# samholt/ODE-Discovery-for-Longitudinal-Heterogeneous-Treatment-Effects-Inference

Measured on AMD Instinct MI355X. Metric: patient-trajectories/sec (N×T RK4 steps) at 1/2/4/8 GPUs; RMSE vs CPU ref, higher is better.
Workload: dtype f64; 1 GPU; C2: PK/PD 100k patients/GPU x 200 steps fp64 - discovery (savgol+FD4+poly2 library+Gram, STLSQ) + RK4 counterfactual rollout; mode=deferred

## Files before the change

ode-discovery-for-longitudinal-heterogeneous-treatment-effects-inference_amd/csrc/insite_common.h:

```cpp
#pragma once
#include <hip/hip_runtime.h>

#include <cstdint>

#include "insite_hip.h"

namespace {

constexpr int kWave = 64;
constexpr int kWavesPerBlock = 4;
constexpr int kBlock = kWave * kWavesPerBlock;

#define SGC(a, b, c, d, e, den) a / den, b / den, c / den, d / den, e / den
__device__ __forceinline__ double dot5(double w0, double w1, double w2, double w3, double w4,
                                       double a, double b, double c, double d, double e) {
  return w0 * a + w1 * b + w2 * c + w3 * d + w4 * e;
}

__device__ __forceinline__ double sg_interior(double a, double b, double c, double d, double e) {
  return dot5(SGC(-3.0, 12.0, 17.0, 12.0, -3.0, 35.0), a, b, c, d, e);
}
__device__ __forceinline__ double sg_pos0(double a, double b, double c, double d, double e) {
  return dot5(SGC(69.0, 4.0, -6.0, 4.0, -1.0, 70.0), a, b, c, d, e);
}
__device__ __forceinline__ double sg_pos1(double a, double b, double c, double d, double e) {
  return dot5(SGC(2.0, 27.0, 12.0, -8.0, 2.0, 35.0), a, b, c, d, e);
}
__device__ __forceinline__ double sg_pos3(double a, double b, double c, double d, double e) {
  return dot5(SGC(2.0, -8.0, 12.0, 27.0, 2.0, 35.0), a, b, c, d, e);
}
__device__ __forceinline__ double sg_pos4(double a, double b, double c, double d, double e) {
  return dot5(SGC(-1.0, 4.0, -6.0, 4.0, 69.0, 70.0), a, b, c, d, e);
}
__device__ __forceinline__ double fd_interior(double a, double b, double , double d, double e) {
  return (1.0 / 12.0) * a + (-2.0 / 3.0) * b + (2.0 / 3.0) * d + (-1.0 / 12.0) * e;
}
__device__ __forceinline__ double fd_pos0(double a, double b, double c, double d, double e) {
  return dot5(-25.0 / 12.0, 4.0, -3.0, 4.0 / 3.0, -0.25, a, b, c, d, e);
}
__device__ __forceinline__ double fd_pos1(double a, double b, double c, double d, double e) {
  return dot5(-0.25, -5.0 / 6.0, 1.5, -0.5, 1.0 / 12.0, a, b, c, d, e);
}
__device__ __forceinline__ double fd_pos3(double a, double b, double c, double d, double e) {
  return dot5(-1.0 / 12.0, 0.5, -1.5, 5.0 / 6.0, 0.25, a, b, c, d, e);
}
__device__ __forceinline__ double fd_pos4(double a, double b, double c, double d, double e) {
  return dot5(0.25, -4.0 / 3.0, 3.0, -4.0, 25.0 / 12.0, a, b, c, d, e);
}

__device__ __forceinline__ void wave_lds_sync() {
  __builtin_amdgcn_fence(__ATOMIC_SEQ_CST, "wavefront");
  __builtin_amdgcn_wave_barrier();
  __builtin_amdgcn_fence(__ATOMIC_SEQ_CST, "wavefront");
}

__device__ __forceinline__ int wave_min_i(int v) {
#pragma unroll
  for (int off = 32; off > 0; off >>= 1) v = min(v, __shfl_xor(v, off, kWave));
  return __builtin_amdgcn_readfirstlane(v);
}
__device__ __forceinline__ int wave_max_i(int v) {
#pragma unroll
  for (int off = 32; off > 0; off >>= 1) v = max(v, __shfl_xor(v, off, kWave));
  return __builtin_amdgcn_readfirstlane(v);
}

__device__ __forceinline__ unsigned bit_transpose32(unsigned x, int lane) {
  const unsigned m[5] = {0x0000FFFFu, 0x00FF00FFu, 0x0F0F0F0Fu, 0x33333333u, 0x55555555u};
#pragma unroll
  for (int k = 0; k < 5; ++k) {
    const int sh = 16 >> k;
    const unsigned y = (unsigned)__shfl_xor((int)x, sh, kWave);
    x = (lane & sh) ? ((x & ~m[k]) | ((y >> sh) & m[k])) : ((x & m[k]) | ((y << sh) & ~m[k]));
  }
  return x;
}

struct GramW {
  double sg0, sg1, sg2;
  double fd1, fd2;
  double inv_dt;
};

__device__ __forceinline__ double sg_int(const GramW& w, double a, double b, double c, double d, double e) {
  return w.sg0 * c + w.sg1 * (b + d) + w.sg2 * (a + e);
}
__device__ __forceinline__ double fd_int(const GramW& w, double a, double b, double d, double e) {
  return w.fd1 * (d - b) + w.fd2 * (e - a);
}

typedef double dbl4 __attribute__((ext_vector_type(4)));
constexpr unsigned kOOB = 0x80000000u;

typedef unsigned int u32x4 __attribute__((ext_vector_type(4)));
typedef unsigned int u32x2 __attribute__((ext_vector_type(2)));

struct StlsqParams {
  double thr, alpha;
  int32_t max_iter, unbias, enabled;
};


#ifndef INSITE_STORE_AUX
#define INSITE_STORE_AUX 2
#endif
constexpr int kStoreAux = INSITE_STORE_AUX;

inline int32_t launch_status() { return hipGetLastError() == hipSuccess ? INSITE_OK : INSITE_E_HIP; }

}
```

ode-discovery-for-longitudinal-heterogeneous-treatment-effects-inference_amd/csrc/insite_hip.hip:

```cpp
#include <hip/hip_runtime.h>
#include <type_traits>

#include <cmath>
#include <cstdint>
#include <atomic>
#include <cstring>

#include "insite_hip.h"
#include "insite_irregular.h"
#include "insite_affine.h"

namespace {

constexpr int kGramMaxBlocks = 1024;
constexpr int kPsStride = 17;

#ifdef INSITE_TIMING
constexpr int kTsWaves = 1 << 16, kTsSlots = 10;
__device__ unsigned long long g_tstamp[kTsWaves * kTsSlots];
#define INSITE_TSTAMP(wave, slot)                                                                   \
  do {                                                                                              \
    const unsigned long long t_ = __builtin_amdgcn_s_memtime();                                     \
    if ((threadIdx.x & 63) == 0 && (wave) < kTsWaves) g_tstamp[(int64_t)(wave) * kTsSlots + (slot)] = t_; \
  } while (0)
// ... 28 lines not shown
  int8_t ex[INSITE_MAX_TERMS];
  int8_t eu[INSITE_MAX_TERMS][INSITE_MAX_STATICS];
  int8_t ei[kMaxEntries];
  int8_t ek[kMaxEntries];
  int32_t mfma;
  int32_t nq;
  int32_t n_atoms;
  int8_t atom_exp[16][INSITE_MAX_STATICS];
  int8_t col_atom[INSITE_MAX_TERMS];
  int8_t qatom[16];
  int8_t qmom[16];
  int8_t qcol[kMaxEntries];
  int32_t ucode[INSITE_MAX_TERMS];
  int32_t acode[16];
};

__device__ __forceinline__ double monomial(const LibDesc& lib, int j, const double* u) {
  return monomial_code(lib.ucode[j] & 0xffffff, u);
}
__device__ __forceinline__ int col_ex(const LibDesc& lib, int j) { return (lib.ucode[j] >> 24) & 0xff; }

#ifndef INSITE_GT
#define INSITE_GT 16
#endif
#ifndef INSITE_PF
#define INSITE_PF 1
#endif
constexpr int kGT = INSITE_GT;
constexpr int kGStride = kGT + 1;
constexpr int kGSlot = kGStride > 17 ? kGStride : 17;
constexpr int kGPF = INSITE_PF;
#ifndef INSITE_GRAM_SCPF
#define INSITE_GRAM_SCPF 1
#endif
#ifndef INSITE_TM_DEPTH
#define INSITE_TM_DEPTH 2
#endif
constexpr int kTmDepth = INSITE_TM_DEPTH;

__device__ __forceinline__ void add_row(double xk, double dk, double& Sx, double& Sxx, double& Sd, double& Sdx) {
  Sx += xk;
  Sxx = fma(xk, xk, Sxx);
  Sd += dk;
  Sdx = fma(dk, xk, Sdx);
}

template <int LL>
__device__ void small_trajectory(const double* __restrict__ xrow, int64_t step, const GramW& w, double& Sx,
                                 double& Sxx, double& Sd, double& Sdx) {
  double xv[LL], xs[LL];
#pragma unroll
  for (int j = 0; j < LL; ++j) xv[j] = xrow[j * step];
#pragma unroll
  for (int k = 0; k < LL; ++k) {
    if (k == 0) xs[k] = sg_pos0(xv[0], xv[1], xv[2], xv[3], xv[4]);
    else if (k == 1) xs[k] = sg_pos1(xv[0], xv[1], xv[2], xv[3], xv[4]);
    else if (k == LL - 2) xs[k] = sg_pos3(xv[LL - 5], xv[LL - 4], xv[LL - 3], xv[LL - 2], xv[LL - 1]);
    else if (k == LL - 1) xs[k] = sg_pos4(xv[LL - 5], xv[LL - 4], xv[LL - 3], xv[LL - 2], xv[LL - 1]);
    else xs[k] = sg_int(w, xv[k - 2], xv[k - 1], xv[k], xv[k + 1], xv[k + 2]);
  }
#pragma unroll
  for (int k = 0; k < LL; ++k) {
    double d;
    if (k == 0) d = fd_pos0(xs[0], xs[1], xs[2], xs[3], xs[4]) * w.inv_dt;
    else if (k == 1) d = fd_pos1(xs[0], xs[1], xs[2], xs[3], xs[4]) * w.inv_dt;
    else if (k == LL - 2) d = fd_pos3(xs[LL - 5], xs[LL - 4], xs[LL - 3], xs[LL - 2], xs[LL - 1]) * w.inv_dt;
    else if (k == LL - 1) d = fd_pos4(xs[LL - 5], xs[LL - 4], xs[LL - 3], xs[LL - 2], xs[LL - 1]) * w.inv_dt;
    else d = fd_int(w, xs[k - 2], xs[k - 1], xs[k + 1], xs[k + 2]);
    add_row(xv[k], d, Sx, Sxx, Sd, Sdx);
  }
}


__device__ __forceinline__ void tele_hi(const GramW& w, double vm1, double v0, double v1, double v2, double& sd,
                                        double& sdx) {
  sd = w.fd1 * (v1 + v0) + w.fd2 * ((v2 + v1) + (v0 + vm1));
  sdx = w.fd1 * (v0 * v1) + w.fd2 * (vm1 * v1 + v0 * v2);
}
__device__ __forceinline__ void tele_lo(const GramW& w, double vm2, double vm1, double v0, double v1, double& sd,
                                        double& sdx) {
  sd = w.fd1 * (v0 + vm1) + w.fd2 * ((v1 + v0) + (vm1 + vm2));
  sdx = w.fd1 * (vm1 * v0) + w.fd2 * (vm2 * v0 + vm1 * v1);
}

#ifndef INSITE_TAIL_RELEASE_FENCE
#define INSITE_TAIL_RELEASE_FENCE 0
#endif
constexpr int kTailGroup = 16;
constexpr int kTailMaxGroups = 64;
constexpr int kTailMaxEnt = INSITE_MAX_ARMS * (INSITE_MAX_TERMS * (INSITE_MAX_TERMS + 1) / 2 + INSITE_MAX_TERMS);
struct GramOut {
  double* G;
  double* b;
  int n_arms;
  double* coef;
  int8_t* mask;
  int32_t* iters;
  StlsqParams sp;
  double* mom;
};

template <int F>
__device__ int stlsq_solve(const double (&g)[F][F], const double (&rhs)[F], double thr, double alpha,
                           int max_iter, int unbias, double (&c)[F], unsigned& sup,
                           unsigned init = (1u << F) - 1u);

__device__ __forceinline__ void tail_store(double* p, double v) {
  __hip_atomic_store(reinterpret_cast<unsigned long long*>(p), __double_as_longlong(v), __ATOMIC_RELAXED,
                     __HIP_MEMORY_SCOPE_AGENT);
}

template <int STF>
__device__ __forceinline__ void tail_finish(double* red, int n_ent, const LibDesc& lib, const GramOut& o) {
  const int64_t F = lib.F;
  double* dense = red + kTailMaxEnt + 8;
  constexpr int kDense = STF * STF + STF;
  for (int idx = threadIdx.x; idx < n_ent; idx += kBlock) {
    const int a = idx / lib.nE, e = idx - a * lib.nE;
    const int i = lib.ei[e], k = lib.ek[e];
    const double v = red[idx];
    if (k >= 0) {
      o.G[(a * F + i) * F + k] = v;
      o.G[(a * F + k) * F + i] = v;
      if constexpr (STF > 0) {
        dense[a * kDense + i * STF + k] = v;
        dense[a * kDense + k * STF + i] = v;
      }
    } else {
      o.b[a * F + i] = v;
      if constexpr (STF > 0) dense[a * kDense + STF * STF + i] = v;
    }
  }
  if constexpr (STF > 0) {
    __syncthreads();
    const int a = (int)threadIdx.x;
    if (a < o.n_arms) {
      const double* d = dense + a * kDense;
      double g[STF][STF], rhs[STF], c[STF];
#pragma unroll
      for (int i = 0; i < STF; ++i) {
        rhs[i] = d[STF * STF + i];
#pragma unroll
        for (int j = 0; j <= i; ++j) g[i][j] = d[i * STF + j];
      }
      unsigned sup = 0u;
      const int it = stlsq_solve<STF>(g, rhs, o.sp.thr, o.sp.alpha, o.sp.max_iter, o.sp.unbias, c, sup);
#pragma unroll
      for (int i = 0; i < STF; ++i) {
        o.coef[a * STF + i] = c[i];
        if (o.mask) o.mask[a * STF + i] = (int8_t)((sup >> i) & 1u);
      }
      if (o.iters) o.iters[a] = it;
    }
  }
}

template <int STF>
__device__ __forceinline__ void gram_tail(const int vblk, const int nblk, double* __restrict__ part, int n_ent,
                                          unsigned* __restrict__ cnt, const LibDesc& lib, const GramOut& o,
                                          double* red) {
  int* flag = reinterpret_cast<int*>(red + kTailMaxEnt);
  const int tg = nblk <= kTailGroup * kTailMaxGroups
                     ? kTailGroup
                     : ((nblk + kTailMaxGroups - 1) / kTailMaxGroups + kTailGroup - 1) / kTailGroup * kTailGroup;
  const int ng = (nblk + tg - 1) / tg;
  const int g = vblk / tg;
// ... 139 lines not shown
          const double2 v = *reinterpret_cast<const double2*>(q);
          vx[j] = v.x;
          vy[j] = v.y;
        } else {
          vx[j] = q[0];
          vy[j] = odd_last ? 0.0 : q[1];
        }
      }
#pragma unroll
      for (int j = 0; j < kDynUnroll; ++j) {
        ax += r + j < r1 ? vx[j] : 0.0;
        ay += r + j < r1 ? vy[j] : 0.0;
      }
    }
    gsum[gq * 2 * npair + 2 * pp] = ax;
    gsum[gq * 2 * npair + 2 * pp + 1] = ay;
  }
  __syncthreads();
  for (int q = t; q < n_ent; q += kBlock) {
    double acc = 0.0;
    for (int g = 0; g < ngr; ++g) acc += gsum[g * 2 * npair + q];
    red[q] = acc;
  }
  __syncthreads();
  tail_finish<STF>(red, n_ent, lib, o);
}
static_assert(kTailMaxEnt + 8 + INSITE_MAX_ARMS * (INSITE_MAX_TERMS * INSITE_MAX_TERMS + INSITE_MAX_TERMS) +
                      2 * kBlock + 64 <= kWavesPerBlock * kWave * kGSlot,
              "dyn_finalize's group sums fit the gram kernel's LDS array");
static_assert(kTailMaxEnt + 8 + INSITE_MAX_ARMS * (INSITE_MAX_TERMS * INSITE_MAX_TERMS + INSITE_MAX_TERMS) <=
                  kWavesPerBlock * kWave * kGSlot,
              "tail scratch fits the gram kernel's LDS array");

constexpr int kGramSmem = kWavesPerBlock * kWave * kGSlot;
#ifndef INSITE_GRAM_ORDER
#define INSITE_GRAM_ORDER 0
#endif
#ifndef INSITE_GRAM_LOAD_AUX
#define INSITE_GRAM_LOAD_AUX 0
#endif
__device__ __forceinline__ int64_t gram_item_tile(int64_t item, int n_seg, int64_t n_tiles) {
  return INSITE_GRAM_ORDER ? item % n_tiles : item / n_seg;
}
__device__ __forceinline__ int gram_item_seg(int64_t item, int n_seg, int64_t n_tiles) {
  return INSITE_GRAM_ORDER ? (int)(item / n_tiles) : (int)(item - (item / n_seg) * n_seg);
}
template <bool MFMA, int NARM>
__device__ __forceinline__ void gram_block_partial(const int vblk, double* __restrict__ smem, const LibDesc& lib,
                                                   const GramOut& out, double* __restrict__ partial, const dbl4& cacc,
                                                   const double (&acc)[NARM], const int wid, const int lane) {
  __syncthreads();
  double* red = smem;
  const int n_ent = out.n_arms * lib.nE;
  if constexpr (MFMA) {
#pragma unroll
    for (int j = 0; j < 4; ++j) red[wid * 256 + ((lane >> 4) + 4 * j) * 16 + (lane & 15)] = cacc[j];
  } else {
#pragma unroll
    for (int a = 0; a < NARM; ++a) red[(wid * NARM + a) * kWave + lane] = acc[a];
  }
  __syncthreads();
  for (int idx = threadIdx.x; idx < n_ent; idx += kBlock) {
    const int a = idx / lib.nE, e = idx - a * lib.nE;
    const int q = MFMA ? (a * lib.F + lib.ei[e]) * 16 + lib.qcol[e] : a * kWave + e;
    constexpr int stride = MFMA ? 256 : NARM * kWave;
    double v = red[q];
#pragma unroll
    for (int ww = 1; ww < kWavesPerBlock; ++ww) v += red[ww * stride + q];
    tail_store(partial + (int64_t)vblk * n_ent + idx, v);
  }
}

template <int VEC, int NARM, bool SMOOTH, bool MFMA, bool TM, int MOM, int STF = 0, int DYN = 0>
__device__ __forceinline__ void gram_body(const int vblk, const int vgrid, double* __restrict__ smem,
            const double* __restrict__ x, int64_t ldx, int n_steps, const double* __restrict__ u,
            const int8_t* __restrict__ arm, const int32_t* __restrict__ rows, int64_t N, int seg, int n_seg,
            const GramW& w, const LibDesc& lib, double* __restrict__ partial, unsigned* __restrict__ cnt,
            const GramOut& out, const DynGram* __restrict__ dgp = nullptr) {
  static_assert(!DYN || (TM && MFMA && MOM == 0), "the claimed gram tail is the deferred step's (time-major, MFMA)");
  const int lane = threadIdx.x & (kWave - 1);
  const int wid = __builtin_amdgcn_readfirstlane(threadIdx.x / kWave);
  double* xt = smem + wid * (kWave * kGSlot);
  constexpr int kMinMain = SMOOTH ? 8 : 5;
  constexpr int kWarm = SMOOTH ? 8 : 4;
  constexpr int kLag = SMOOTH ? 4 : 2;
  constexpr int LPR = kGT / VEC;
  constexpr int RPI = kWave / LPR;
  constexpr int NLD = kWave / RPI;
  static_assert(!TM || (VEC == 1 && NLD == kGT), "time-major tiles hold the lane's own kGT samples");
  INSITE_TSTAMP(blockIdx.x * kWavesPerBlock + wid, 0);
  INSITE_TREAL(blockIdx.x * kWavesPerBlock + wid, 8);
  INSITE_THWID(blockIdx.x * kWavesPerBlock + wid);

  dbl4 cacc = {0.0, 0.0, 0.0, 0.0};
  double acc[NARM];
#pragma unroll
  for (int a = 0; a < NARM; ++a) acc[a] = 0.0;
  const int my_i = lane < lib.nE ? lib.ei[lane] : 0;
  const int my_k = lane < lib.nE ? lib.ek[lane] : 0;
  const int my_exi = lib.ex[my_i];
  const int my_exk = my_k >= 0 ? lib.ex[my_k] : 0;
  const int pr_r = lane & 15;
  const int pr_a = pr_r / lib.F, pr_i = pr_r - (pr_r / lib.F) * lib.F;
  const bool pr_ok = MFMA && pr_r < NARM * lib.F;
  const int pr_atom = pr_ok ? lib.col_atom[pr_i] : 0;
  const bool q_ok = MFMA && pr_r < lib.nq;
  const int q_atom = q_ok ? lib.qatom[pr_r] : 0;
  const int q_mom = q_ok ? lib.qmom[pr_r] : 0;
  const int cl = (lane % LPR) * VEC;

  const int64_t n_tiles = (N + kWave - 1) / kWave;
  const bool ranged = n_seg == 0;
  const int ng = (n_steps + kGT - 1) / kGT;
  const int64_t nW = (int64_t)vgrid * kWavesPerBlock;
  const int64_t wv = (int64_t)vblk * kWavesPerBlock + wid;
  const int64_t units = ranged ? n_tiles * ng : n_tiles * n_seg;
  const int64_t units_s = (DYN && ranged) ? dgp->tile0 * ng : units;
  const int64_t c_end = ranged ? (wv + 1) * units_s / nW : units;
  struct Piece {
    int64_t tile, next;
    int s0, sE;
  };
  auto piece_of = [&](int64_t c) -> Piece {
    Piece pc;
    if (ranged) {
      pc.tile = c / ng;
      const int g0 = (int)(c - pc.tile * ng);
      const int g1 = (int)min((int64_t)ng, (int64_t)g0 + (c_end - c));
      pc.s0 = g0 * kGT;
      pc.sE = g1 * kGT;
      pc.next = c + (g1 - g0);
    } else {
      pc.tile = gram_item_tile(c, n_seg, n_tiles);
      pc.s0 = gram_item_seg(c, n_seg, n_tiles) * seg;
      pc.sE = pc.s0 + seg;
      pc.next = c + nW;
    }
    return pc;
  };
  typedef double TmTile[kGT];
  TmTile vr[TM ? kTmDepth : 1];
  bool prefetched = false;
  int sc_L = 0, sc_a = -1;
  double sc_u[INSITE_MAX_STATICS] = {0.0, 0.0, 0.0};
  auto sc_load = [&](int64_t pp) {
    const int64_t pcl = pp < N ? pp : N - 1;
    sc_L = rows[pcl];
    sc_a = arm[pcl];
#pragma unroll
    for (int t = 0; t < INSITE_MAX_STATICS; ++t) sc_u[t] = u[pcl * lib.U + (t < lib.U ? t : 0)];
  };
  auto tm_load_for = [&](TmTile& v, int t0, int lim, int64_t q0, int qv, unsigned qoff) {
    const int nrow = lim - t0 < kGT ? lim - t0 : kGT;
    const int bytes = nrow > 0 ? (int)(((int64_t)(nrow - 1) * ldx + qv) * 8) : 0;
    const __amdgpu_buffer_rsrc_t rs = __builtin_amdgcn_make_buffer_rsrc(
        (void*)(x + (int64_t)(nrow > 0 ? t0 : 0) * ldx + q0), (short)0, bytes, 0x00020000);
#pragma unroll
    for (int i = 0; i < kGT; ++i)
      v[i] = __builtin_bit_cast(double, __builtin_amdgcn_raw_buffer_load_b64(rs, qoff + (unsigned)(i * ldx * 8), 0,
                                                                             INSITE_GRAM_LOAD_AUX));
  };
  int64_t dq = -1, dnext = -1;
  bool dnext_ok = false, dinfl = false, dexh = !DYN || dgp->P <= 0;
  int dphase = 0, dh = (int)(blockIdx.x % kDynHeads), dtried = 0;
  unsigned dcl = 0u, dmine = 0u;
  auto dyn_issue = [&]() {
    if constexpr (DYN) {
      if (lane == 0) dcl = __hip_atomic_fetch_add(dgp->claim + dh * kClaimWords, 1u, __ATOMIC_RELAXED,
                                                  __HIP_MEMORY_SCOPE_AGENT);
      dinfl = true;
    }
  };
  auto dyn_read = [&]() -> int64_t {
    if constexpr (DYN) {
      for (;;) {
        const int64_t idx = (int64_t)__builtin_amdgcn_readfirstlane(dcl);
        const int64_t lo = dh * dgp->P / kDynHeads, hi = (dh + 1) * dgp->P / kDynHeads;
        dinfl = false;
        if (lo + idx < hi) return lo + idx;
        if (++dtried >= kDynHeads) {
          dexh = true;
          return -1;
        }
        dh = (dh + 1) % kDynHeads;
        dyn_issue();
      }
    }
    return -1;
  };
  auto dyn_piece = [&](int64_t q) -> Piece {
    Piece pc;
    const int64_t tt = q / dgp->ppt;
    const int j = (int)(q - tt * dgp->ppt);
    pc.tile = dgp->tile0 + tt;
    pc.s0 = j * dgp->pg * kGT;
    pc.sE = min(ng, (j + 1) * dgp->pg) * kGT;
    pc.next = 0;
    return pc;
  };
  int64_t cur = ranged ? wv * units_s / nW : wv;
  for (;;) {
    Piece pc;
    if (cur < c_end) {
      pc = piece_of(cur);
      cur = pc.next;
      if constexpr (DYN)
        if (!(cur < c_end) && !dexh) dyn_issue();
    } else {
      if constexpr (!DYN) {
        break;
      } else {
        if (dphase == 0) {
          gram_block_partial<MFMA, NARM>(vblk, smem, lib, out, partial, cacc, acc, wid, lane);
          __syncthreads();
          cacc = {0.0, 0.0, 0.0, 0.0};
          dphase = 1;
        } else {
          wave_lds_sync();
#pragma unroll
          for (int j = 0; j < 4; ++j) xt[((lane >> 4) + 4 * j) * 16 + (lane & 15)] = cacc[j];
          wave_lds_sync();
          const int n_ent = out.n_arms * lib.nE;
          for (int idx = lane; idx < n_ent; idx += kWave) {
            const int a = idx / lib.nE, e = idx - a * lib.nE;
            dgp->ppart[dq * n_ent + idx] = xt[(a * lib.F + lib.ei[e]) * 16 + lib.qcol[e]];
          }
          wave_lds_sync();
          cacc = {0.0, 0.0, 0.0, 0.0};
        }
        if (!dnext_ok) {
          if (!dinfl && !dexh) dyn_issue();
          dnext = dinfl ? dyn_read() : -1;
        }
        dnext_ok = false;
        dq = dnext;
        if (dq < 0) break;
        ++dmine;
        pc = dyn_piece(dq);
        if (!dexh) dyn_issue();
      }
    }
    const int64_t tile = pc.tile;
    const int64_t p0 = tile * kWave;
    const int64_t p = p0 + lane;
    const int s0 = pc.s0;
    const bool first = s0 == 0;
    const int tb = first ? 0 : s0 - kWarm;
    const int tm_valid = (int)(N - p0 < kWave ? N - p0 : kWave);
    const unsigned tm_off = p < N ? (unsigned)lane * 8u : kOOB;
    auto tm_load = [&](TmTile& v, int t0, int lim) { tm_load_for(v, t0, lim, p0, tm_valid, tm_off); };
    if (!(TM && INSITE_GRAM_SCPF && prefetched)) sc_load(p);
#ifndef INSITE_GRAM_LATE_ISSUE
    if constexpr (TM) {
      const int s1p = min(pc.sE, n_steps);
      if (!prefetched) {
#pragma unroll
        for (int d = 0; d < kTmDepth; ++d)
          if (tb + d * kGT < s1p) tm_load(vr[d], tb + d * kGT, s1p);
      }
    }
#endif
    prefetched = false;
    int L = 0;
    int arm_p = -1;
    double uu[INSITE_MAX_STATICS] = {0.0, 0.0, 0.0};
    {
      const int Lr = sc_L;
      const int ar = sc_a;
#pragma unroll
      for (int t = 0; t < INSITE_MAX_STATICS; ++t) uu[t] = (p < N && t < lib.U) ? sc_u[t] : 0.0;
      if (p < N) {
        L = Lr;
        arm_p = ar;
        if (L > n_steps) L = n_steps;
        if (L < 5) L = 0;
      }
    }
    const int Lm = L >= kMinMain ? L : 0;
    const int Lmax = wave_max_i(Lm);
    const int s1 = min(pc.sE, Lmax);
    INSITE_TSTAMP(blockIdx.x * kWavesPerBlock + wid, 1);
    const int e = min(Lm, pc.sE);
    const int Lmin = wave_min_i(e);
    const int bstart = max(2 * kLag, s0);
    const bool has_body = e > bstart;
    double Sx = 0.0, Sxx = 0.0, Sd = 0.0, Sdx = 0.0;

    if (s0 < Lmax) {
      typedef double TileRegs[NLD][VEC];
      TileRegs vA, vB;
      auto load_tile = [&](TileRegs& v, int t0) {
        const int col = t0 + cl;
        const bool col_ok = col < s1;
        const int colc = col_ok ? col : 0;
#pragma unroll
        for (int it = 0; it < NLD; ++it) {
          const int64_t pr = p0 + it * RPI + lane / LPR;
          const bool ok = col_ok && pr < N;
          const double* src = x + (pr < N ? pr : N - 1) * ldx + colc;
          if constexpr (VEC == 2) {
            const double2 q = *reinterpret_cast<const double2*>(src);
            v[it][0] = ok ? q.x : 0.0;
            v[it][1] = ok ? q.y : 0.0;
          } else {
            const double q = *src;
            v[it][0] = ok ? q : 0.0;
          }
        }
      };
      auto store_tile = [&](const TileRegs& v) {
        if constexpr (TM) return;
        wave_lds_sync();
#pragma unroll
        for (int it = 0; it < NLD; ++it) {
          const int r = it * RPI + lane / LPR;
#pragma unroll
          for (int q = 0; q < VEC; ++q) xt[r * kGStride + cl + q] = v[it][q];
        }
        wave_lds_sync();
      };

      double xr[8], sr[8];
#pragma unroll
      for (int j = 0; j < 8; ++j) xr[j] = sr[j] = 0.0;
      double loSd = 0.0, loSdx = 0.0;
      const bool tail = Lm > 0 && e == Lm && Lm - 1 >= s0;
      const bool need_end = has_body || tail;
      constexpr int NQ = SMOOTH ? 8 : 5;
      double qe[NQ];
      bool tail_issued = false;
      auto issue_tail = [&]() {
        if (tail_issued) return;
        tail_issued = true;
        const int64_t pc = p < N ? p : N - 1;
        const double* xe = TM ? x + (need_end ? (int64_t)(e - NQ) * ldx + pc : pc)
                              : x + (need_end ? p * ldx + (e - NQ) : 0);
        const int64_t st = TM ? (need_end ? ldx : 0) : 1;
#pragma unroll
        for (int j = 0; j < NQ; ++j) {
          const double q = xe[j * st];
          qe[j] = need_end ? q : 0.0;
        }
      };

      auto sample = [&](const auto& v, int i) -> double {
        if constexpr (TM) return v[i];
        else return xt[lane * kGStride + i];
      };
      if constexpr (TM) {
#ifdef INSITE_GRAM_LATE_ISSUE
#pragma unroll
        for (int d = 0; d < kTmDepth; ++d)
          if (tb + d * kGT < s1) tm_load(vr[d], tb + d * kGT, s1);
#endif
        if (!(tb + kTmDepth * kGT < s1)) issue_tail();
      } else {
        load_tile(vA, tb);
        store_tile(vA);
        if (tb + kGT < s1) load_tile(vA, tb + kGT);
        if constexpr (kGPF == 2) {
          if (tb + 2 * kGT < s1) load_tile(vB, tb + 2 * kGT);
          else issue_tail();
        } else {
          if (tb + kGT >= s1) issue_tail();
        }
      }
      {
        const bool masked = tb + kGT > Lmin;
#pragma unroll
        for (int i = 0; i < kGT; ++i) {
          if constexpr (TM) xr[i & 7] = sample(vr[0], i);
          else xr[i & 7] = sample(vA, i);
          const int t = tb + i;
          if constexpr (SMOOTH) {
            if (i >= 4) sr[(i - 2) & 7] = sg_int(w, xr[(i - 4) & 7], xr[(i - 3) & 7], xr[(i - 2) & 7], xr[(i - 1) & 7], xr[i & 7]);
            if (i == 7) {
              if (first) {
                const double xs0 = sg_pos0(xr[0], xr[1], xr[2], xr[3], xr[4]);
                const double xs1 = sg_pos1(xr[0], xr[1], xr[2], xr[3], xr[4]);
                const double d0 = fd_pos0(xs0, xs1, sr[2], sr[3], sr[4]) * w.inv_dt;
                const double d1 = fd_pos1(xs0, xs1, sr[2], sr[3], sr[4]) * w.inv_dt;
                const double d2 = fd_int(w, xs0, xs1, sr[3], sr[4]);
                const double d3 = fd_int(w, xs1, sr[2], sr[4], sr[5]);
                const bool on = Lm > 0;
                add_row(on ? xr[0] : 0.0, on ? d0 : 0.0, Sx, Sxx, Sd, Sdx);
                add_row(on ? xr[1] : 0.0, on ? d1 : 0.0, Sx, Sxx, Sd, Sdx);
                add_row(on ? xr[2] : 0.0, on ? d2 : 0.0, Sx, Sxx, Sd, Sdx);
                add_row(on ? xr[3] : 0.0, on ? d3 : 0.0, Sx, Sxx, Sd, Sdx);
              }
            }
            if (i >= 8) {
              double xk = xr[(i - 4) & 7];
              double dk = fd_int(w, sr[(i - 6) & 7], sr[(i - 5) & 7], sr[(i - 3) & 7], sr[(i - 2) & 7]);
              if (masked) {
                xk = (t < e) ? xk : 0.0;
                dk = (t < e) ? dk : 0.0;
              }
              add_row(xk, dk, Sx, Sxx, Sd, Sdx);
            }
          } else {
            if (i == 3) tele_lo(w, xr[0], xr[1], xr[2], xr[3], loSd, loSdx);
            if (i == 4 && first) {
              const double d0 = fd_pos0(xr[0], xr[1], xr[2], xr[3], xr[4]) * w.inv_dt;
              const double d1 = fd_pos1(xr[0], xr[1], xr[2], xr[3], xr[4]) * w.inv_dt;
              const bool on = Lm > 0;
              add_row(on ? xr[0] : 0.0, on ? d0 : 0.0, Sx, Sxx, Sd, Sdx);
              add_row(on ? xr[1] : 0.0, on ? d1 : 0.0, Sx, Sxx, Sd, Sdx);
            }
            if (i >= 4) {
              double xk = xr[(i - 2) & 7];
              if (masked) xk = (t < e) ? xk : 0.0;
              Sx += xk;
              Sxx = fma(xk, xk, Sxx);
            }
          }
        }
      }
      INSITE_TSTAMP(blockIdx.x * kWavesPerBlock + wid, 2);
      auto consume = [&](int t0, const auto& v) {
        if (t0 + kGT <= Lmin) {
#ifdef INSITE_ABLATE_GRAM_NOCOMPUTE
#pragma unroll
          for (int i = 0; i < kGT; ++i) Sx += sample(v, i);
          return;
#endif
#pragma unroll
          for (int i = 0; i < kGT; ++i) {
            xr[i & 7] = sample(v, i);
            if constexpr (SMOOTH) {
              sr[(i - 2) & 7] = sg_int(w, xr[(i - 4) & 7], xr[(i - 3) & 7], xr[(i - 2) & 7], xr[(i - 1) & 7], xr[i & 7]);
              add_row(xr[(i - 4) & 7], fd_int(w, sr[(i - 6) & 7], sr[(i - 5) & 7], sr[(i - 3) & 7], sr[(i - 2) & 7]),
                      Sx, Sxx, Sd, Sdx);
            } else {
              const double xk = xr[(i - 2) & 7];
              Sx += xk;
              Sxx = fma(xk, xk, Sxx);
            }
          }
        } else {
#pragma unroll
          for (int i = 0; i < kGT; ++i) {
            if (t0 + i < s1) {
              xr[i & 7] = sample(v, i);
              const bool own = t0 + i < e;
              if constexpr (SMOOTH) {
                sr[(i - 2) & 7] = sg_int(w, xr[(i - 4) & 7], xr[(i - 3) & 7], xr[(i - 2) & 7], xr[(i - 1) & 7], xr[i & 7]);
                const double dk = fd_int(w, sr[(i - 6) & 7], sr[(i - 5) & 7], sr[(i - 3) & 7], sr[(i - 2) & 7]);
                add_row(own ? xr[(i - 4) & 7] : 0.0, own ? dk : 0.0, Sx, Sxx, Sd, Sdx);
              } else {
                const double xk = own ? xr[(i - 2) & 7] : 0.0;
                Sx += xk;
                Sxx = fma(xk, xk, Sxx);
              }
            }
          }
        }
      };
      if constexpr (TM) {
        if (tb + kTmDepth * kGT < s1) tm_load(vr[0], tb + kTmDepth * kGT, s1);
        else issue_tail();
        for (int t0 = tb + kGT; t0 < s1;) {
#pragma unroll
          for (int d = 1; d <= kTmDepth; ++d) {
            if (t0 < s1) {
              consume(t0, vr[d % kTmDepth]);
              if (t0 + kTmDepth * kGT < s1) tm_load(vr[d % kTmDepth], t0 + kTmDepth * kGT, s1);
              else issue_tail();
              t0 += kGT;
            }
          }
        }
#ifndef INSITE_GRAM_NO_XPREFETCH
        {
          bool have = cur < c_end;
          Piece np;
          if (have) {
            np = piece_of(cur);
          } else if constexpr (DYN) {
            if (dinfl) {
              dnext = dyn_read();
              dnext_ok = true;
              have = dnext >= 0;
              if (have) np = dyn_piece(dnext);
            }
          }
          if (have) {
            const int64_t np0 = np.tile * kWave;
            const int ntb = np.s0 == 0 ? 0 : np.s0 - kWarm;
            const int ns1p = min(np.sE, n_steps);
            const int nvalid = (int)(N - np0 < kWave ? N - np0 : kWave);
            const unsigned noff = np0 + lane < N ? (unsigned)lane * 8u : kOOB;
            if (INSITE_GRAM_SCPF) sc_load(np0 + lane);
#pragma unroll
            for (int d = 0; d < kTmDepth; ++d)
              if (ntb + d * kGT < ns1p) tm_load_for(vr[d], ntb + d * kGT, ns1p, np0, nvalid, noff);
            prefetched = true;
          }
        }
#endif
      } else if constexpr (kGPF == 2) {
        for (int t0 = tb + kGT; t0 < s1;) {
          store_tile(vA);
          if (t0 + 2 * kGT < s1) load_tile(vA, t0 + 2 * kGT);
          else issue_tail();
          consume(t0, vA);
          t0 += kGT;
          if (t0 >= s1) break;
          store_tile(vB);
          if (t0 + 2 * kGT < s1) load_tile(vB, t0 + 2 * kGT);
          else issue_tail();
          consume(t0, vB);
          t0 += kGT;
        }
      } else {
        for (int t0 = tb + kGT; t0 < s1; t0 += kGT) {
          store_tile(vA);
          if (t0 + kGT < s1) load_tile(vA, t0 + kGT);
          else issue_tail();
          consume(t0, vA);
        }
      }
      INSITE_TSTAMP(blockIdx.x * kWavesPerBlock + wid, 3);
      issue_tail();
      if (need_end) {
        if constexpr (SMOOTH) {
          const double* q = qe;
          const double a0 = sg_int(w, q[0], q[1], q[2], q[3], q[4]);
          const double a1 = sg_int(w, q[1], q[2], q[3], q[4], q[5]);
          const double a2 = sg_int(w, q[2], q[3], q[4], q[5], q[6]);
          const double a3 = sg_int(w, q[3], q[4], q[5], q[6], q[7]);
          if (tail) {
            const double a4 = sg_pos3(q[3], q[4], q[5], q[6], q[7]);
            const double a5 = sg_pos4(q[3], q[4], q[5], q[6], q[7]);
            add_row(q[4], fd_int(w, a0, a1, a3, a4), Sx, Sxx, Sd, Sdx);
            add_row(q[5], fd_int(w, a1, a2, a4, a5), Sx, Sxx, Sd, Sdx);
            add_row(q[6], fd_pos3(a1, a2, a3, a4, a5) * w.inv_dt, Sx, Sxx, Sd, Sdx);
            add_row(q[7], fd_pos4(a1, a2, a3, a4, a5) * w.inv_dt, Sx, Sxx, Sd, Sdx);
          }
        } else {
          const double* q = qe;
          if (has_body) {
            double hiSd, hiSdx;
            tele_hi(w, q[1], q[2], q[3], q[4], hiSd, hiSdx);
            Sd += hiSd - loSd;
            Sdx += hiSdx - loSdx;
          }
          if (tail) {
            add_row(q[3], fd_pos3(q[0], q[1], q[2], q[3], q[4]) * w.inv_dt, Sx, Sxx, Sd, Sdx);
            add_row(q[4], fd_pos4(q[0], q[1], q[2], q[3], q[4]) * w.inv_dt, Sx, Sxx, Sd, Sdx);
          }
        }
      }
    }
    if constexpr (SMOOTH) {
      if (first && L > 0 && L < kMinMain) {
        const double* xrow = TM ? x + p : x + p * ldx;
        const int64_t st = TM ? ldx : 1;
        if (L == 5) small_trajectory<5>(xrow, st, w, Sx, Sxx, Sd, Sdx);
        else if (L == 6) small_trajectory<6>(xrow, st, w, Sx, Sxx, Sd, Sdx);
        else small_trajectory<7>(xrow, st, w, Sx, Sxx, Sd, Sdx);
      }
    }
    if (s0 >= Lmax && !((SMOOTH || MOM != 0) && first)) continue;
    if constexpr (MOM != 0) {
      if (p < N) {
        double* mrow = (MOM == 1 ? partial : out.mom) + p * 5;
        mrow[0] = (double)L;
        mrow[1] = Sx;
        mrow[2] = Sxx;
        mrow[3] = Sd;
        mrow[4] = Sdx;
      }
      if constexpr (MOM == 1) continue;
    }
#ifdef INSITE_ABLATE_NOGPHASE
    acc[0] += Sx + Sxx + Sd + Sdx;
    continue;
#endif

    INSITE_TSTAMP(blockIdx.x * kWavesPerBlock + wid, 4);
    const double M0 = first ? (double)L : 0.0;
    const int my_arm = (L > 0) ? arm_p : -1;
    double* ps = xt;
    if constexpr (MFMA) {
      constexpr int kRS = 23;
      for (int h = 0; h < 2; ++h) {
        wave_lds_sync();
        if ((lane >> 5) == h) {
          double* row = ps + (lane & 31) * kRS;
          for (int a = 0; a < lib.n_atoms; ++a) {
            const int c = lib.acode[a];
            const int e0 = c & 0xff, e1 = (c >> 8) & 0xff, e2 = (c >> 16) & 0xff;
            double m = 1.0;
            if (e0 >= 1) m *= uu[0];
            if (e0 >= 2) m *= uu[0];
            if (e1 >= 1) m *= uu[1];
            if (e1 >= 2) m *= uu[1];
            if (e2 >= 1) m *= uu[2];
            if (e2 >= 2) m *= uu[2];
            row[a] = m;
          }
          row[16] = M0;
          row[17] = Sx;
          row[18] = Sxx;
          row[19] = Sd;
          row[20] = Sdx;
          row[21] = (double)my_arm;
        }
        wave_lds_sync();
#pragma unroll
        for (int st = 0; st < 8; ++st) {
          const double* row = ps + (4 * st + (lane >> 4)) * kRS;
          const double av = (pr_ok && (int)row[21] == pr_a) ? row[pr_atom] : 0.0;
          const double bv = q_ok ? row[q_atom] * row[16 + q_mom] : 0.0;
          cacc = __builtin_amdgcn_mfma_f64_16x16x4f64(av, bv, cacc, 0, 0, 0);
        }
      }
      wave_lds_sync();
    } else {
      wave_lds_sync();
      for (int j = 0; j < lib.F; ++j) ps[lane * kPsStride + j] = monomial(lib, j, uu);
      ps[lane * kPsStride + 9] = M0;
      ps[lane * kPsStride + 10] = Sx;
      ps[lane * kPsStride + 11] = Sxx;
      ps[lane * kPsStride + 12] = Sd;
      ps[lane * kPsStride + 13] = Sdx;
      ps[lane * kPsStride + 14] = (double)my_arm;
      wave_lds_sync();
      if (lane < lib.nE) {
        const int moff = my_k >= 0 ? 9 + my_exi + my_exk : 12 + my_exi;
        for (int q = 0; q < kWave; ++q) {
          const double* row = ps + q * kPsStride;
          double wq = row[my_i] * row[moff];
          if (my_k >= 0) wq *= row[my_k];
          const int a = (int)row[14];
// ... 2724 lines not shown
static_assert(1 + (kGramMaxBlocks + kTailGroup - 1) / kTailGroup <= kStepRcnt && (kStepRcnt + 2) * sizeof(unsigned) <= kGramWsHeader,
              "step kernel claim counters sit in the header, clear of the gram tail's");

inline int sse_grid(int64_t n_rows) {
  int64_t g = (n_rows + 63) / 64;
  if (g < 1) g = 1;
  if (g > 1024) g = 1024;
  return (int)g;
}


struct GramLaunch {
  const double* x;
  int64_t ldx;
  int n_steps;
  const double* u;
  const int8_t* arm;
  const int32_t* rows;
  int64_t N;
  GramW w;
  LibDesc lib;
  double* part;
  unsigned* cnt;
  GramOut out;
};

#ifndef INSITE_GRAM_RANGED
#define INSITE_GRAM_RANGED 1
#endif
template <int VEC, int NARM, bool SMOOTH, bool MFMA, bool TM, int MOM = 0, int STF = 0>
int launch_gram4(hipStream_t st, const GramLaunch& g) {
  auto kern = gram_kernel<VEC, NARM, SMOOTH, MFMA, TM, MOM, STF>;
  GramPlan pl = gram_plan(g.N, g.n_steps, resident_waves(kern));
  if constexpr (MOM != 0) {
    const int64_t tiles = (g.N + kWave - 1) / kWave;
    const int64_t gres = resident_waves(kern) / kWavesPerBlock;
    int64_t gb = (tiles + kWavesPerBlock - 1) / kWavesPerBlock;
    if (gb > gres && gres > 0) gb = gres;
    pl.grid = (int)(gb < 1 ? 1 : gb);
    pl.n_seg = 1;
    pl.seg = (int)((g.n_steps + kGT - 1) / kGT * kGT);
    if (pl.seg < kGT) pl.seg = kGT;
  } else if (INSITE_GRAM_RANGED && TM) {
    const int64_t units = (g.N + kWave - 1) / kWave * ((g.n_steps + kGT - 1) / kGT);
    int64_t gb = resident_waves(kern) / kWavesPerBlock;
    if (gb > (units + kWavesPerBlock - 1) / kWavesPerBlock) gb = (units + kWavesPerBlock - 1) / kWavesPerBlock;
    if (gb > kGramMaxBlocks) gb = kGramMaxBlocks;
    pl.grid = (int)(gb < 1 ? 1 : gb);
    pl.seg = 0;
    pl.n_seg = 0;
  }
  kern<<<dim3(pl.grid), kBlock, 0, st>>>(g.x, g.ldx, g.n_steps, g.u, g.arm, g.rows, g.N, pl.seg, pl.n_seg, g.w,
                                          g.lib, g.part, g.cnt, g.out);
  return pl.grid;
}

template <int NARM, bool SMOOTH, bool MFMA>
int launch_gram3(int mode, hipStream_t st, const GramLaunch& g) {
  if (mode == 3) return launch_gram4<1, NARM, SMOOTH, MFMA, true, 0, 7>(st, g);
  if (mode == 4) return launch_gram4<1, NARM, SMOOTH, MFMA, true, 2, 7>(st, g);
  if (mode == 5) return launch_gram4<1, NARM, SMOOTH, MFMA, true, 2>(st, g);
  if (mode == 6) return launch_gram4<1, NARM, SMOOTH, MFMA, false, 2>(st, g);
  if (mode == 2) return launch_gram4<1, NARM, SMOOTH, MFMA, true>(st, g);
  if (mode == 1) return launch_gram4<2, NARM, SMOOTH, MFMA, false>(st, g);
  return launch_gram4<1, NARM, SMOOTH, MFMA, false>(st, g);
}

template <int NARM>
int launch_gram(int mode, bool smooth, hipStream_t st, const GramLaunch& g) {
  if (g.lib.mfma) {
    return smooth ? launch_gram3<NARM, true, true>(mode, st, g) : launch_gram3<NARM, false, true>(mode, st, g);
  }
  return smooth ? launch_gram3<NARM, true, false>(mode, st, g) : launch_gram3<NARM, false, false>(mode, st, g);
}

inline GramW make_gram_w(double dt) {
  GramW w;
  w.sg0 = 17.0 / 35.0;
  w.sg1 = 12.0 / 35.0;
  w.sg2 = -3.0 / 35.0;
  w.inv_dt = 1.0 / dt;
  w.fd1 = (2.0 / 3.0) * w.inv_dt;
  w.fd2 = (-1.0 / 12.0) * w.inv_dt;
  return w;
}

template <bool SMOOTH>
int launch_moments(int mode, hipStream_t st, const GramLaunch& g) {
  if (mode == 2) return launch_gram4<1, 1, SMOOTH, false, true, 1>(st, g);
  if (mode == 1) return launch_gram4<2, 1, SMOOTH, false, false, 1>(st, g);
  return launch_gram4<1, 1, SMOOTH, false, false, 1>(st, g);
}

int32_t run_discovery(const double* x, int64_t ldx, int32_t layout, int32_t n_steps, const double* u,
                      const int8_t* arm, const int32_t* rows, int64_t n_patients, int32_t n_statics, int32_t n_arms,
                      const int8_t* exps, int32_t n_terms, int32_t fd_kind, double dt, double* G_out, double* b_out,
                      void* workspace, size_t workspace_bytes, void* stream, const StlsqParams& sp,
                      double* coef_out, int8_t* mask_out, int32_t* iters_out, double* mom_out = nullptr) {
  const bool tm = layout == INSITE_LAYOUT_TIME_MAJOR;
  if (layout != INSITE_LAYOUT_PATIENT_MAJOR && !tm) return INSITE_E_INVALID_ARG;
  if (n_patients < 0 || !G_out || !b_out || n_arms < 1 || n_arms > INSITE_MAX_ARMS || ldx < 1 || !(dt > 0.0) ||
      n_steps < 0 || (tm ? ldx < n_patients : ldx < n_steps))
    return INSITE_E_INVALID_ARG;
  if (n_patients > 0 && (!x || !arm || !rows || (n_statics > 0 && !u))) return INSITE_E_INVALID_ARG;
  if (fd_kind != INSITE_FD_SMOOTHED4 && fd_kind != INSITE_FD_ORDER4) return INSITE_E_UNSUPPORTED;
  LibDesc lib;
  int32_t st = build_lib(exps, n_terms, n_statics, &lib);
  if (st != INSITE_OK) return st;
  if (workspace_bytes < insite_gram_workspace_bytes(n_patients, n_arms, n_terms) || !workspace)
    return INSITE_E_WORKSPACE;
  hipStream_t hs = reinterpret_cast<hipStream_t>(stream);
  const int na = narm_pad(n_arms);
  if (na * lib.F > 16) lib.mfma = 0;
  unsigned* cnt = static_cast<unsigned*>(workspace);
  double* part = reinterpret_cast<double*>(static_cast<char*>(workspace) + kGramWsHeader);
  if (tm && ldx > ((int64_t)1 << 31) / (8 * kGT)) return INSITE_E_UNSUPPORTED;
  const bool vec2 = (ldx % 2 == 0) && ((reinterpret_cast<uintptr_t>(x) & 15u) == 0);
  const int mode = tm ? 2 : (vec2 ? 1 : 0);
  const bool smooth = fd_kind == INSITE_FD_SMOOTHED4;
  if (n_statics == 0) u = x;
#ifdef INSITE_GRAM_MEMSET
  if (hipMemsetAsync(cnt, 0, kGramWsHeader, hs) != hipSuccess) return INSITE_E_HIP;
#endif
#ifndef INSITE_STLSQ_SEPARATE
  const bool fused = sp.enabled && tm && n_terms == 7;
#else
  const bool fused = false;
#endif
  const GramLaunch g{x, ldx, n_steps, u, arm, rows, n_patients, make_gram_w(dt), lib, part, cnt,
                     GramOut{G_out, b_out, n_arms, coef_out, mask_out, iters_out, sp, mom_out}};
  int lmode = fused ? 3 : mode;
  if (mom_out) {
    if (!lib.mfma) return INSITE_E_UNSUPPORTED;
    lmode = tm ? (fused ? 4 : 5) : 6;
  }
  if (na == 1) launch_gram<1>(lmode, smooth, hs, g);
  else if (na == 2) launch_gram<2>(lmode, smooth, hs, g);
  else launch_gram<4>(lmode, smooth, hs, g);
  st = launch_status();
  if (st != INSITE_OK || !sp.enabled || fused) return st;
  switch (n_terms) {
#define INSITE_STL_CASE(FF)                                                                             \
  case FF:                                                                                              \
    stlsq_kernel<FF><<<1, kBlock, 0, hs>>>(G_out, b_out, n_arms, sp.thr, sp.alpha, sp.max_iter, sp.unbias, \
                                           coef_out, mask_out, iters_out);                              \
    break;
    INSITE_STL_CASE(1)
    INSITE_STL_CASE(2)
    INSITE_STL_CASE(3)
    INSITE_STL_CASE(4)
    INSITE_STL_CASE(5)
    INSITE_STL_CASE(6)
    INSITE_STL_CASE(7)
    INSITE_STL_CASE(8)
    INSITE_STL_CASE(9)
#undef INSITE_STL_CASE
    default:
      return INSITE_E_UNSUPPORTED;
  }
  return launch_status();
}

inline int64_t seg_grid(int64_t N) {
  int64_t g = ((N + kWave - 1) / kWave + kWavesPerBlock - 1) / kWavesPerBlock;
  if (g > kSegMaxBlocks) g = kSegMaxBlocks;
  return g < 1 ? 1 : g;
// ... 948 lines not shown
```

Before: 1.557 billion patient-trajectories/s.

## Telescope smoothed-derivative Gram sums to head/tail boundary terms

Extends the telescoping identity already used for the unsmoothed path to the Savitzky-Golay-smoothed path. The composite SG+FD4 stencil coefficients are folded into four constants, so the interior sums of d and d*x reduce to closed-form head and tail terms over eight samples. The main loop then accumulates only Sx and Sxx, and the warm-up overlap between segments (kWarm) is dropped. This removes per-sample stencil arithmetic and re-read of halo samples, at the cost of extra boundary logic and different floating-point rounding in the derivative sums.

```diff
diff --git a/ode-discovery-for-longitudinal-heterogeneous-treatment-effects-inference_amd/csrc/insite_common.h b/ode-discovery-for-longitudinal-heterogeneous-treatment-effects-inference_amd/csrc/insite_common.h
--- a/ode-discovery-for-longitudinal-heterogeneous-treatment-effects-inference_amd/csrc/insite_common.h
+++ b/ode-discovery-for-longitudinal-heterogeneous-treatment-effects-inference_amd/csrc/insite_common.h
@@ -80,7 +80,14 @@
   double sg0, sg1, sg2;
   double fd1, fd2;
   double inv_dt;
+  double c1, c2, c3, c4;
 };
+inline void gram_w_composite(GramW& w) {
+  w.c1 = w.fd1 * w.sg0 + w.fd2 * w.sg1 - w.fd1 * w.sg2;
+  w.c2 = w.fd1 * w.sg1 + w.fd2 * w.sg0;
+  w.c3 = w.fd1 * w.sg2 + w.fd2 * w.sg1;
+  w.c4 = w.fd2 * w.sg2;
+}
 
 __device__ __forceinline__ double sg_int(const GramW& w, double a, double b, double c, double d, double e) {
   return w.sg0 * c + w.sg1 * (b + d) + w.sg2 * (a + e);
diff --git a/ode-discovery-for-longitudinal-heterogeneous-treatment-effects-inference_amd/csrc/insite_hip.hip b/ode-discovery-for-longitudinal-heterogeneous-treatment-effects-inference_amd/csrc/insite_hip.hip
--- a/ode-discovery-for-longitudinal-heterogeneous-treatment-effects-inference_amd/csrc/insite_hip.hip
+++ b/ode-discovery-for-longitudinal-heterogeneous-treatment-effects-inference_amd/csrc/insite_hip.hip
@@ -134,6 +134,25 @@
   sd = w.fd1 * (v0 + vm1) + w.fd2 * ((v1 + v0) + (vm1 + vm2));
   sdx = w.fd1 * (vm1 * v0) + w.fd2 * (vm2 * v0 + vm1 * v1);
 }
+__device__ __forceinline__ void tele9_end(const GramW& w, const double (&v)[8], double& sd, double& sdx) {
+  const double s1 = v[3] + v[4];
+  const double s2 = s1 + (v[2] + v[5]);
+  const double s3 = s2 + (v[1] + v[6]);
+  const double s4 = s3 + (v[0] + v[7]);
+  sd = (w.c1 * s1 + w.c2 * s2) + (w.c3 * s3 + w.c4 * s4);
+  sdx = (w.c1 * (v[3] * v[4]) + w.c2 * (v[2] * v[4] + v[3] * v[5])) +
+        (w.c3 * (v[1] * v[4] + v[2] * v[5] + v[3] * v[6]) + w.c4 * ((v[0] * v[4] + v[1] * v[5]) + (v[2] * v[6] + v[3] * v[7])));
+}
+__device__ __forceinline__ void tele9_hi(const GramW& w, const double (&xe)[8], double& sd, double& sdx) {
+  tele9_end(w, xe, sd, sdx);
+}
+__device__ __forceinline__ void tele9_lo(const GramW& w, const double (&xh)[8], double& sd, double& sdx) {
+  tele9_end(w, xh, sd, sdx);
+}
+__device__ __forceinline__ void add_drow(double xk, double dk, double& Sd, double& Sdx) {
+  Sd += dk;
+  Sdx = fma(dk, xk, Sdx);
+}
 
 #ifndef INSITE_TAIL_RELEASE_FENCE
 #define INSITE_TAIL_RELEASE_FENCE 0
@@ -439,8 +458,8 @@
   const int wid = __builtin_amdgcn_readfirstlane(threadIdx.x / kWave);
   double* xt = smem + wid * (kWave * kGSlot);
   constexpr int kMinMain = SMOOTH ? 8 : 5;
-  constexpr int kWarm = SMOOTH ? 8 : 4;
-  constexpr int kLag = SMOOTH ? 4 : 2;
+  constexpr int kEdge = SMOOTH ? 4 : 2;
+  static_assert(kGT >= kMinMain, "the first tile holds the head samples x[0 .. kMinMain)");
   constexpr int LPR = kGT / VEC;
   constexpr int RPI = kWave / LPR;
   constexpr int NLD = kWave / RPI;
@@ -602,7 +621,7 @@
     const int64_t p = p0 + lane;
     const int s0 = pc.s0;
     const bool first = s0 == 0;
-    const int tb = first ? 0 : s0 - kWarm;
+    const int tb = s0;
     const int tm_valid = (int)(N - p0 < kWave ? N - p0 : kWave);
     const unsigned tm_off = p < N ? (unsigned)lane * 8u : kOOB;
     auto tm_load = [&](TmTile& v, int t0, int lim) { tm_load_for(v, t0, lim, p0, tm_valid, tm_off); };
@@ -639,8 +658,6 @@
     INSITE_TSTAMP(blockIdx.x * kWavesPerBlock + wid, 1);
     const int e = min(Lm, pc.sE);
     const int Lmin = wave_min_i(e);
-    const int bstart = max(2 * kLag, s0);
-    const bool has_body = e > bstart;
     double Sx = 0.0, Sxx = 0.0, Sd = 0.0, Sdx = 0.0;
 
     if (s0 < Lmax) {
@@ -677,17 +694,18 @@
         wave_lds_sync();
       };
 
-      double xr[8], sr[8];
-#pragma unroll
-      for (int j = 0; j < 8; ++j) xr[j] = sr[j] = 0.0;
+      const bool body = Lm > 2 * kEdge;
       double loSd = 0.0, loSdx = 0.0;
       const bool tail = Lm > 0 && e == Lm && Lm - 1 >= s0;
-      const bool need_end = has_body || tail;
-      constexpr int NQ = SMOOTH ? 8 : 5;
+      const bool need_end = tail;
+      const bool any_tail = __builtin_amdgcn_ballot_w64(tail) != 0;
+      constexpr int NQ = kMinMain;
       double qe[NQ];
+#pragma unroll
+      for (int j = 0; j < NQ; ++j) qe[j] = 0.0;
       bool tail_issued = false;
       auto issue_tail = [&]() {
-        if (tail_issued) return;
+        if (tail_issued || !any_tail) return;
         tail_issued = true;
         const int64_t pc = p < N ? p : N - 1;
         const double* xe = TM ? x + (need_end ? (int64_t)(e - NQ) * ldx + pc : pc)
@@ -722,97 +740,67 @@
           if (tb + kGT >= s1) issue_tail();
         }
       }
-      {
-        const bool masked = tb + kGT > Lmin;
-#pragma unroll
-        for (int i = 0; i < kGT; ++i) {
-          if constexpr (TM) xr[i & 7] = sample(vr[0], i);
-          else xr[i & 7] = sample(vA, i);
-          const int t = tb + i;
-          if constexpr (SMOOTH) {
-            if (i >= 4) sr[(i - 2) & 7] = sg_int(w, xr[(i - 4) & 7], xr[(i - 3) & 7], xr[(i - 2) & 7], xr[(i - 1) & 7], xr[i & 7]);
-            if (i == 7) {
-              if (first) {
-                const double xs0 = sg_pos0(xr[0], xr[1], xr[2], xr[3], xr[4]);
-                const double xs1 = sg_pos1(xr[0], xr[1], xr[2], xr[3], xr[4]);
-                const double d0 = fd_pos0(xs0, xs1, sr[2], sr[3], sr[4]) * w.inv_dt;
-                const double d1 = fd_pos1(xs0, xs1, sr[2], sr[3], sr[4]) * w.inv_dt;
-                const double d2 = fd_int(w, xs0, xs1, sr[3], sr[4]);
-                const double d3 = fd_int(w, xs1, sr[2], sr[4], sr[5]);
-                const bool on = Lm > 0;
-                add_row(on ? xr[0] : 0.0, on ? d0 : 0.0, Sx, Sxx, Sd, Sdx);
-                add_row(on ? xr[1] : 0.0, on ? d1 : 0.0, Sx, Sxx, Sd, Sdx);
-                add_row(on ? xr[2] : 0.0, on ? d2 : 0.0, Sx, Sxx, Sd, Sdx);
-                add_row(on ? xr[3] : 0.0, on ? d3 : 0.0, Sx, Sxx, Sd, Sdx);
-              }
-            }
-            if (i >= 8) {
-              double xk = xr[(i - 4) & 7];
-              double dk = fd_int(w, sr[(i - 6) & 7], sr[(i - 5) & 7], sr[(i - 3) & 7], sr[(i - 2) & 7]);
-              if (masked) {
-                xk = (t < e) ? xk : 0.0;
-                dk = (t < e) ? dk : 0.0;
-              }
-              add_row(xk, dk, Sx, Sxx, Sd, Sdx);
-            }
-          } else {
-            if (i == 3) tele_lo(w, xr[0], xr[1], xr[2], xr[3], loSd, loSdx);
-            if (i == 4 && first) {
-              const double d0 = fd_pos0(xr[0], xr[1], xr[2], xr[3], xr[4]) * w.inv_dt;
-              const double d1 = fd_pos1(xr[0], xr[1], xr[2], xr[3], xr[4]) * w.inv_dt;
-              const bool on = Lm > 0;
-              add_row(on ? xr[0] : 0.0, on ? d0 : 0.0, Sx, Sxx, Sd, Sdx);
-              add_row(on ? xr[1] : 0.0, on ? d1 : 0.0, Sx, Sxx, Sd, Sdx);
-            }
-            if (i >= 4) {
-              double xk = xr[(i - 2) & 7];
-              if (masked) xk = (t < e) ? xk : 0.0;
+      auto consume = [&](int t0, const auto& v) {
+        if (t0 + kGT <= Lmin) {
+#ifdef INSITE_ABLATE_GRAM_NOCOMPUTE
+#pragma unroll
+          for (int i = 0; i < kGT; ++i) Sx += sample(v, i);
+          return;
+#endif
+#pragma unroll
+          for (int i = 0; i < kGT; ++i) {
+            const double xk = sample(v, i);
+            Sx += xk;
+            Sxx = fma(xk, xk, Sxx);
+          }
+        } else {
+#pragma unroll
+          for (int i = 0; i < kGT; ++i) {
+            if (t0 + i < s1) {
+              const double xk = (t0 + i < e) ? sample(v, i) : 0.0;
               Sx += xk;
               Sxx = fma(xk, xk, Sxx);
             }
           }
         }
-      }
+      };
+      auto first_tile = [&](const auto& v) {
+        if (first) {
+          double h[kMinMain];
+#pragma unroll
+          for (int i = 0; i < kMinMain; ++i) h[i] = sample(v, i);
+          const bool on = Lm > 0;
+          if constexpr (SMOOTH) {
+            const double xs0 = sg_pos0(h[0], h[1], h[2], h[3], h[4]);
+            const double xs1 = sg_pos1(h[0], h[1], h[2], h[3], h[4]);
+            const double xs2 = sg_int(w, h[0], h[1], h[2], h[3], h[4]);
+            const double xs3 = sg_int(w, h[1], h[2], h[3], h[4], h[5]);
+            const double xs4 = sg_int(w, h[2], h[3], h[4], h[5], h[6]);
+            const double xs5 = sg_int(w, h[3], h[4], h[5], h[6], h[7]);
+            const double d0 = fd_pos0(xs0, xs1, xs2, xs3, xs4) * w.inv_dt;
+            const double d1 = fd_pos1(xs0, xs1, xs2, xs3, xs4) * w.inv_dt;
+            const double d2 = fd_int(w, xs0, xs1, xs3, xs4);
+            const double d3 = fd_int(w, xs1, xs2, xs4, xs5);
+            add_drow(on ? h[0] : 0.0, on ? d0 : 0.0, Sd, Sdx);
+            add_drow(on ? h[1] : 0.0, on ? d1 : 0.0, Sd, Sdx);
+            add_drow(on ? h[2] : 0.0, on ? d2 : 0.0, Sd, Sdx);
+            add_drow(on ? h[3] : 0.0, on ? d3 : 0.0, Sd, Sdx);
+            tele9_lo(w, h, loSd, loSdx);
+          } else {
+            const double d0 = fd_pos0(h[0], h[1], h[2], h[3], h[4]) * w.inv_dt;
+            const double d1 = fd_pos1(h[0], h[1], h[2], h[3], h[4]) * w.inv_dt;
+            add_drow(on ? h[0] : 0.0, on ? d0 : 0.0, Sd, Sdx);
+            add_drow(on ? h[1] : 0.0, on ? d1 : 0.0, Sd, Sdx);
+            tele_lo(w, h[0], h[1], h[2], h[3], loSd, loSdx);
+          }
+          loSd = body ? loSd : 0.0;
+          loSdx = body ? loSdx : 0.0;
+        }
+        consume(tb, v);
+      };
+      if constexpr (TM) first_tile(vr[0]);
+      else first_tile(vA);
       INSITE_TSTAMP(blockIdx.x * kWavesPerBlock + wid, 2);
-      auto consume = [&](int t0, const auto& v) {
-        if (t0 + kGT <= Lmin) {
-#ifdef INSITE_ABLATE_GRAM_NOCOMPUTE
-#pragma unroll
-          for (int i = 0; i < kGT; ++i) Sx += sample(v, i);
-          return;
-#endif
-#pragma unroll
-          for (int i = 0; i < kGT; ++i) {
-            xr[i & 7] = sample(v, i);
-            if constexpr (SMOOTH) {
-              sr[(i - 2) & 7] = sg_int(w, xr[(i - 4) & 7], xr[(i - 3) & 7], xr[(i - 2) & 7], xr[(i - 1) & 7], xr[i & 7]);
-              add_row(xr[(i - 4) & 7], fd_int(w, sr[(i - 6) & 7], sr[(i - 5) & 7], sr[(i - 3) & 7], sr[(i - 2) & 7]),
-                      Sx, Sxx, Sd, Sdx);
-            } else {
-              const double xk = xr[(i - 2) & 7];
-              Sx += xk;
-              Sxx = fma(xk, xk, Sxx);
-            }
-          }
-        } else {
-#pragma unroll
-          for (int i = 0; i < kGT; ++i) {
-            if (t0 + i < s1) {
-              xr[i & 7] = sample(v, i);
-              const bool own = t0 + i < e;
-              if constexpr (SMOOTH) {
-                sr[(i - 2) & 7] = sg_int(w, xr[(i - 4) & 7], xr[(i - 3) & 7], xr[(i - 2) & 7], xr[(i - 1) & 7], xr[i & 7]);
-                const double dk = fd_int(w, sr[(i - 6) & 7], sr[(i - 5) & 7], sr[(i - 3) & 7], sr[(i - 2) & 7]);
-                add_row(own ? xr[(i - 4) & 7] : 0.0, own ? dk : 0.0, Sx, Sxx, Sd, Sdx);
-              } else {
-                const double xk = own ? xr[(i - 2) & 7] : 0.0;
-                Sx += xk;
-                Sxx = fma(xk, xk, Sxx);
-              }
-            }
-          }
-        }
-      };
       if constexpr (TM) {
         if (tb + kTmDepth * kGT < s1) tm_load(vr[0], tb + kTmDepth * kGT, s1);
         else issue_tail();
@@ -843,7 +831,7 @@
           }
           if (have) {
             const int64_t np0 = np.tile * kWave;
-            const int ntb = np.s0 == 0 ? 0 : np.s0 - kWarm;
+            const int ntb = np.s0;
             const int ns1p = min(np.sE, n_steps);
             const int nvalid = (int)(N - np0 < kWave ? N - np0 : kWave);
             const unsigned noff = np0 + lane < N ? (unsigned)lane * 8u : kOOB;
@@ -879,35 +867,30 @@
       }
       INSITE_TSTAMP(blockIdx.x * kWavesPerBlock + wid, 3);
       issue_tail();
-      if (need_end) {
+      double hiSd = 0.0, hiSdx = 0.0;
+      if (tail) {
         if constexpr (SMOOTH) {
           const double* q = qe;
           const double a0 = sg_int(w, q[0], q[1], q[2], q[3], q[4]);
           const double a1 = sg_int(w, q[1], q[2], q[3], q[4], q[5]);
           const double a2 = sg_int(w, q[2], q[3], q[4], q[5], q[6]);
           const double a3 = sg_int(w, q[3], q[4], q[5], q[6], q[7]);
-          if (tail) {
-            const double a4 = sg_pos3(q[3], q[4], q[5], q[6], q[7]);
-            const double a5 = sg_pos4(q[3], q[4], q[5], q[6], q[7]);
-            add_row(q[4], fd_int(w, a0, a1, a3, a4), Sx, Sxx, Sd, Sdx);
-            add_row(q[5], fd_int(w, a1, a2, a4, a5), Sx, Sxx, Sd, Sdx);
-            add_row(q[6], fd_pos3(a1, a2, a3, a4, a5) * w.inv_dt, Sx, Sxx, Sd, Sdx);
-            add_row(q[7], fd_pos4(a1, a2, a3, a4, a5) * w.inv_dt, Sx, Sxx, Sd, Sdx);
-          }
+          const double a4 = sg_pos3(q[3], q[4], q[5], q[6], q[7]);
+          const double a5 = sg_pos4(q[3], q[4], q[5], q[6], q[7]);
+          add_drow(q[4], fd_int(w, a0, a1, a3, a4), Sd, Sdx);
+          add_drow(q[5], fd_int(w, a1, a2, a4, a5), Sd, Sdx);
+          add_drow(q[6], fd_pos3(a1, a2, a3, a4, a5) * w.inv_dt, Sd, Sdx);
+          add_drow(q[7], fd_pos4(a1, a2, a3, a4, a5) * w.inv_dt, Sd, Sdx);
+          if (body) tele9_hi(w, qe, hiSd, hiSdx);
         } else {
           const double* q = qe;
-          if (has_body) {
-            double hiSd, hiSdx;
-            tele_hi(w, q[1], q[2], q[3], q[4], hiSd, hiSdx);
-            Sd += hiSd - loSd;
-            Sdx += hiSdx - loSdx;
-          }
-          if (tail) {
-            add_row(q[3], fd_pos3(q[0], q[1], q[2], q[3], q[4]) * w.inv_dt, Sx, Sxx, Sd, Sdx);
-            add_row(q[4], fd_pos4(q[0], q[1], q[2], q[3], q[4]) * w.inv_dt, Sx, Sxx, Sd, Sdx);
-          }
+          add_drow(q[3], fd_pos3(q[0], q[1], q[2], q[3], q[4]) * w.inv_dt, Sd, Sdx);
+          add_drow(q[4], fd_pos4(q[0], q[1], q[2], q[3], q[4]) * w.inv_dt, Sd, Sdx);
+          if (body) tele_hi(w, q[1], q[2], q[3], q[4], hiSd, hiSdx);
         }
       }
+      Sd += hiSd - loSd;
+      Sdx += hiSdx - loSdx;
     }
     if constexpr (SMOOTH) {
       if (first && L > 0 && L < kMinMain) {
@@ -3798,6 +3781,7 @@
   w.inv_dt = 1.0 / dt;
   w.fd1 = (2.0 / 3.0) * w.inv_dt;
   w.fd2 = (-1.0 / 12.0) * w.inv_dt;
+  gram_w_composite(w);
   return w;
 }
 
```

New measurement: 1.584 billion patient-trajectories/s, median of 6. No clear change (+1.8%).
